# david-zwicker/video-analysis

Measured on AMD Instinct MI355X. Metric: frames/sec (bg-sub+blur+thresh+CCL) 1080p uint8, higher is better.
Workload: dtype u8; 1 GPU; cfg3_1080p_full_chain: 1920x1080 uint8, batch 256/GPU, running-mean bg-sub (f64 state) + sigma=5 Gaussian (q8.8) + threshold 20 + 5x5 dilate/erode + 4-connected labelling + object counts; inputs resident in HBM; engine=bg=1 gauss=mfma-i8(ksize=31) thresh=20 morph=2 ccl=4, video=one clip per rank, overlap=off, world_size=1, backend=single process

## Files before the change

video-analysis_amd/csrc/va_morph.hip:

```cpp
#include <math.h>

#include "va_common.h"

namespace va {

int make_row_spans(int shape, int ksize, RowSpans *out)
{
    VA_REQUIRE(ksize >= 1, "morphology: ksize must be >= 1 (got %d)", ksize);
    if (ksize > 63) {
        set_error("morphology: ksize %d > 63 is not supported", ksize);
        return VA_ERR_RANGE;
    }
    VA_REQUIRE(shape >= VA_SHAPE_RECT && shape <= VA_SHAPE_ELLIPSE, "morphology: bad shape %d",
               shape);
    out->ksize = ksize;
    out->anchor = ksize / 2;
    const int r = ksize / 2, c = ksize / 2;
    const double inv_r2 = r ? 1.0 / ((double)r * r) : 0.0;
    for (int i = 0; i < ksize; i++) {
        int j1 = 0, j2 = 0;
        if (shape == VA_SHAPE_RECT || (shape == VA_SHAPE_CROSS && i == r)) {
            j2 = ksize;
        } else if (shape == VA_SHAPE_CROSS) {
            j1 = c;
            j2 = j1 + 1;
        } else {
            int dy = i - r;
            if (abs(dy) <= r) {
                int dx = (int)lrint(c * sqrt((r * r - dy * dy) * inv_r2));
                j1 = c - dx > 0 ? c - dx : 0;
                j2 = c + dx + 1 < ksize ? c + dx + 1 : ksize;
            }
        }
        out->lo[i] = (int8_t)j1;
        out->hi[i] = (int8_t)j2;
    }
    return VA_OK;
}

namespace {

constexpr int kBlock = 256;

__global__ void __launch_bounds__(kBlock)
pack_bits_kernel(const uint8_t *__restrict__ src, uint32_t *__restrict__ bits, int w, int w32,
                 size_t total_words, int thresh, int vec_ok)
{
    size_t t = (size_t)blockIdx.x * kBlock + threadIdx.x;
    if (t >= total_words)
        return;
    int wi = (int)(t % w32);
    size_t rowi = t / w32;
    const uint8_t *p = src + rowi * (size_t)w + (size_t)wi * 32;
    int nvalid = w - wi * 32;
    nvalid = nvalid > 32 ? 32 : nvalid;
    uint32_t m = 0;
    if (vec_ok && nvalid == 32) {
        uint4 a = reinterpret_cast<const uint4 *>(p)[0];
        uint4 b = reinterpret_cast<const uint4 *>(p)[1];
        uint8_t px[32];
        memcpy(px, &a, 16);
        memcpy(px + 16, &b, 16);
#pragma unroll
        for (int k = 0; k < 32; k++)
            m |= (uint32_t)((int)px[k] > thresh) << k;
    } else {
        for (int k = 0; k < nvalid; k++)
            m |= (uint32_t)((int)p[k] > thresh) << k;
    }
    bits[t] = m;
}

__global__ void __launch_bounds__(kBlock)
unpack_bits_wide_kernel(const uint32_t *__restrict__ bits, uint8_t *__restrict__ dst, size_t total_halves,
                        int maxval)
{
    const size_t t = (size_t)blockIdx.x * kBlock + threadIdx.x;
    if (t >= total_halves)
        return;
    const uint32_t m = (bits[t >> 1] >> (16 * (t & 1))) & 0xFFFFu;
    typedef unsigned int v4u __attribute__((ext_vector_type(4)));
    v4u v;
#pragma unroll
    for (int q = 0; q < 4; q++)
        v[q] = ((((m >> (4 * q)) & 0xFu) * 0x00204081u) & 0x01010101u) * (uint32_t)maxval;
    __builtin_nontemporal_store(v, reinterpret_cast<v4u *>(dst + 16 * t));
}

__global__ void __launch_bounds__(kBlock)
unpack_bits_kernel(const uint32_t *__restrict__ bits, uint8_t *__restrict__ dst, int w, int w32,
                   size_t total_words, int maxval, int vec_ok)
{
    size_t t = (size_t)blockIdx.x * kBlock + threadIdx.x;
    if (t >= total_words)
        return;
    int wi = (int)(t % w32);
    size_t rowi = t / w32;
    uint8_t *p = dst + rowi * (size_t)w + (size_t)wi * 32;
    int nvalid = w - wi * 32;
    nvalid = nvalid > 32 ? 32 : nvalid;
    uint32_t m = bits[t];
    if (vec_ok && nvalid == 32) {
        uint8_t px[32];
#pragma unroll
        for (int k = 0; k < 32; k++)
            px[k] = (m >> k) & 1u ? (uint8_t)maxval : (uint8_t)0;
        uint4 a, b;
        memcpy(&a, px, 16);
        memcpy(&b, px + 16, 16);
        reinterpret_cast<uint4 *>(p)[0] = a;
        reinterpret_cast<uint4 *>(p)[1] = b;
    } else {
        for (int k = 0; k < nvalid; k++)
            p[k] = (m >> k) & 1u ? (uint8_t)maxval : (uint8_t)0;
    }
}

template <bool DILATE>
__global__ void __launch_bounds__(kBlock)
morph_bits_kernel(const uint32_t *__restrict__ src, uint32_t *__restrict__ dst, int h, int w,
                  int w32, size_t total_words, RowSpans se)
{
    size_t t = (size_t)blockIdx.x * kBlock + threadIdx.x;
    if (t >= total_words)
        return;
    const int wi = (int)(t % w32);
    const size_t rowi = t / w32;
    const int y = (int)(rowi % h);
    const uint32_t *frame = src + (rowi - y) * (size_t)w32;
    const uint32_t border = DILATE ? 0u : 0xFFFFFFFFu;
    const int tail = w & 31;
    const uint32_t last_valid = tail ? (0xFFFFFFFFu >> (32 - tail)) : 0xFFFFFFFFu;
    uint32_t acc = border;
    for (int i = 0; i < se.ksize; i++) {
        const int yy = y + i - se.anchor;
        if (yy < 0 || yy >= h)
            continue;
        const int lo = se.lo[i] - se.anchor, hi = se.hi[i] - 1 - se.anchor;
        if (lo > hi)
            continue;
        const uint32_t *row = frame + (size_t)yy * w32;
        uint32_t c = row[wi];
        uint32_t l = wi > 0 ? row[wi - 1] : border;
        uint32_t r = wi + 1 < w32 ? row[wi + 1] : border;
        if (!DILATE) {
            if (wi == w32 - 1)
                c |= ~last_valid;
            if (wi + 1 == w32 - 1)
                r |= ~last_valid;
        }
        uint32_t racc = border;
        for (int dx = lo; dx <= hi; dx++) {
            uint32_t s;
            if (dx == 0)
                s = c;
            else if (dx > 0)
                s = (c >> dx) | (r << (32 - dx));
            else
                s = (c << -dx) | (l >> (32 + dx));
            racc = DILATE ? (racc | s) : (racc & s);
        }
        acc = DILATE ? (acc | racc) : (acc & racc);
    }
    if (wi == w32 - 1)
        acc &= last_valid;
    dst[t] = acc;
}

struct MorphSeq {
    int count;
    int reach_total;
    int op[VA_MAX_MORPH_OPS];
    RowSpans se[VA_MAX_MORPH_OPS];
};
constexpr int kBandRows = 32;

__device__ __forceinline__ uint32_t morph_word_lds(const uint32_t *buf, int rbase, int y, int wi,
                                                  int h, int w32, uint32_t last_valid,
                                                  const RowSpans &se, bool dilate)
{
    const uint32_t border = dilate ? 0u : 0xFFFFFFFFu;
    uint32_t acc = border;
    for (int i = 0; i < se.ksize; i++) {
        const int yy = y + i - se.anchor;
        if (yy < 0 || yy >= h)
            continue;
        const int lo = se.lo[i] - se.anchor, hi = se.hi[i] - 1 - se.anchor;
        if (lo > hi)
            continue;
        const uint32_t *row = buf + (size_t)(yy - rbase) * w32;
        uint32_t c = row[wi];
        uint32_t l = wi > 0 ? row[wi - 1] : border;
        uint32_t r = wi + 1 < w32 ? row[wi + 1] : border;
        if (!dilate) {
            if (wi == w32 - 1)
                c |= ~last_valid;
            if (wi + 1 == w32 - 1)
                r |= ~last_valid;
        }
        uint32_t racc = border;
        for (int dx = lo; dx <= hi; dx++) {
            uint32_t sft;
            if (dx == 0)
                sft = c;
            else if (dx > 0)
                sft = (c >> dx) | (r << (32 - dx));
            else
                sft = (c << -dx) | (l >> (32 + dx));
            racc = dilate ? (racc | sft) : (racc & sft);
        }
        acc = dilate ? (acc | racc) : (acc & racc);
    }
    if (wi == w32 - 1)
        acc &= last_valid;
    return acc;
}

__device__ __forceinline__ uint32_t shift_words(uint32_t l, uint32_t c, uint32_t r, int dx)
{
    if (dx == 0)
        return c;
    return dx > 0 ? __builtin_amdgcn_alignbit(r, c, dx) : __builtin_amdgcn_alignbit(c, l, 32 + dx);
}

__global__ void __launch_bounds__(kBlock)
morph_fused_kernel(const uint32_t *__restrict__ src, uint32_t *__restrict__ dst, int h, int w, int w32, int nbands, MorphSeq seq)
{
    extern __shared__ uint32_t s_rows[];
    const int band = blockIdx.x % nbands, f = blockIdx.x / nbands;
    const int tx = threadIdx.x & 63, ty = threadIdx.x >> 6;
    const int y0 = band * kBandRows;
    const int nrows = kBandRows + 2 * seq.reach_total;
    const int rbase = y0 - seq.reach_total;
    uint32_t *bufA = s_rows, *bufB = s_rows + (size_t)nrows * w32, *bufH = bufB + (size_t)nrows * w32;
    const uint32_t *fsrc = src + (size_t)f * h * w32;
    const int tail = w & 31;
    const uint32_t last_valid = tail ? (0xFFFFFFFFu >> (32 - tail)) : 0xFFFFFFFFu;

    for (int wi = tx; wi < w32; wi += 64) {
        for (int r0 = ty; r0 < nrows; r0 += 32) {
            uint32_t tmp[8];
#pragma unroll
            for (int j = 0; j < 8; j++) {
                const int r = r0 + 4 * j, y = rbase + r;
                tmp[j] = (r < nrows && y >= 0 && y < h) ? fsrc[(size_t)y * w32 + wi] : 0u;
            }
#pragma unroll
            for (int j = 0; j < 8; j++) {
                const int r = r0 + 4 * j;
                if (r < nrows)
                    bufA[r * w32 + wi] = tmp[j];
            }
        }
    }
    __syncthreads();

    int reach = 0;
    for (int k = 0; k < seq.count; k++) {
        const RowSpans &se = seq.se[k];
        const int a = se.anchor, b = se.ksize - 1 - se.anchor;
        reach += a > b ? a : b;
        const int lo = max(0, rbase + reach), hi = min(h, rbase + nrows - reach);
        const bool dil = seq.op[k] == VA_MORPH_DILATE;
        const uint32_t border = dil ? 0u : 0xFFFFFFFFu;
        bool rect = true;
        for (int i = 1; i < se.ksize; i++)
            rect = rect && se.lo[i] == se.lo[0] && se.hi[i] == se.hi[0];
        rect = rect && se.lo[0] < se.hi[0];
        if (rect) {
            const int dlo = se.lo[0] - a, dhi = se.hi[0] - 1 - a;
            const int ylo = max(0, lo - a), yhi = min(h, hi + b);
            for (int y = ylo + ty; y < yhi; y += 4) {
                const uint32_t *row = bufA + (y - rbase) * w32;
                for (int wi = tx; wi < w32; wi += 64) {
                    uint32_t c = row[wi];
                    uint32_t l = wi > 0 ? row[wi - 1] : border;
                    uint32_t r = wi + 1 < w32 ? row[wi + 1] : border;
                    if (!dil) {
                        if (wi == w32 - 1)
                            c |= ~last_valid;
                        if (wi + 1 == w32 - 1)
                            r |= ~last_valid;
                    }
                    uint32_t racc = border;
                    for (int dx = dlo; dx <= dhi; dx++) {
                        const uint32_t sft = shift_words(l, c, r, dx);
                        racc = dil ? (racc | sft) : (racc & sft);
                    }
                    bufH[(y - rbase) * w32 + wi] = racc;
                }
            }
            __syncthreads();
            for (int y = lo + ty; y < hi; y += 4) {
                const int i0 = max(0, a - y), i1 = min(se.ksize, h + a - y);
                for (int wi = tx; wi < w32; wi += 64) {
                    uint32_t acc = border;
                    for (int i = i0; i < i1; i++) {
                        const uint32_t v = bufH[(y + i - a - rbase) * w32 + wi];
                        acc = dil ? (acc | v) : (acc & v);
                    }
                    if (wi == w32 - 1)
                        acc &= last_valid;
                    bufB[(y - rbase) * w32 + wi] = acc;
                }
            }
        } else {
            for (int y = lo + ty; y < hi; y += 4)
                for (int wi = tx; wi < w32; wi += 64)
                    bufB[(y - rbase) * w32 + wi] =
                        morph_word_lds(bufA, rbase, y, wi, h, w32, last_valid, se, dil);
        }
        __syncthreads();
        uint32_t *t = bufA;
        bufA = bufB;
        bufB = t;
    }

    const int yend = min(h, y0 + kBandRows);
    uint32_t *fdst = dst + (size_t)f * h * w32;
    for (int y = y0 + ty; y < yend; y += 4) {
        const uint32_t *row = bufA + (y - rbase) * w32;
        for (int wi = tx; wi < w32; wi += 64)
            fdst[(size_t)y * w32 + wi] = row[wi];
    }
}

constexpr int kStreamBand = 32;

template <int K>
__device__ __forceinline__ uint32_t hdilate(uint32_t l, uint32_t c, uint32_t r)
{
    uint32_t acc = c;
#pragma unroll
    for (int d = 1; d <= K / 2; d++) {
        acc |= __builtin_amdgcn_alignbit(r, c, d);
        acc |= __builtin_amdgcn_alignbit(c, l, 32 - d);
    }
    return acc;
}

constexpr int kStreamGroup = 8;

__device__ __forceinline__ uint32_t lane_left(uint32_t v)
{
    return __builtin_amdgcn_update_dpp(0u, v, 0x138 , 0xf, 0xf, true);
}
__device__ __forceinline__ uint32_t lane_right(uint32_t v)
{
    return __builtin_amdgcn_update_dpp(0u, v, 0x130 , 0xf, 0xf, true);
}

template <int K0, int K1>
__global__ void __launch_bounds__(kBlock)
morph_stream_kernel(const uint32_t *__restrict__ src, uint32_t *__restrict__ dst, int n, int h, int w,
                     int w32, int nbands, int nchunks, uint32_t flip_in, uint32_t flip_mid,
                     uint32_t flip_out)
{
    constexpr int A0 = K0 / 2, A1 = K1 / 2;
    constexpr int LO = K1 ? 2 : 1;
    constexpr int COLS = K1 ? 60 : 62;
    const int lane = threadIdx.x & 63;
    size_t item = (size_t)blockIdx.x * (kBlock / 64) + (threadIdx.x >> 6);
    const int chunk = (int)(item % nchunks);
    item /= nchunks;
    const int band = (int)(item % nbands);
    const size_t f = item / nbands;
    if (f >= (size_t)n)
        return;
    const int wi = chunk * COLS + lane - LO;
    const bool col_in = wi >= 0 && wi < w32;
    const bool col_store = col_in && lane >= LO && lane < LO + COLS;
    const int tail = w & 31;
    const uint32_t valid = !col_in ? 0u : (wi == w32 - 1 && tail ? (0xFFFFFFFFu >> (32 - tail)) : 0xFFFFFFFFu);
    const uint32_t *fsrc = src + f * (size_t)h * w32 + min(max(wi, 0), w32 - 1);
    uint32_t *fdst = dst + f * (size_t)h * w32;

    const int y0 = band * kStreamBand;
    if (y0 >= h)
        return;
    const int y_first = y0 - A0 - A1;
    const int y_last = min(h, y0 + kStreamBand) - 1 + A0 + A1;

    auto load_group = [&](int y, uint32_t (&g)[kStreamGroup]) {
#pragma unroll
        for (int k = 0; k < kStreamGroup; k++)
            g[k] = fsrc[(size_t)min(max(y + k, 0), h - 1) * w32];
#pragma unroll
        for (int k = 0; k < kStreamGroup; k++)
            g[k] = (y + k >= 0 && y + k < h) ? ((g[k] ^ flip_in) & valid) : 0u;
    };

    uint32_t win0[K0], win1[K1 ? K1 : 1];
#pragma unroll
    for (int k = 0; k < K0; k++)
        win0[k] = 0u;
#pragma unroll
    for (int k = 0; k < (K1 ? K1 : 1); k++)
        win1[k] = 0u;

    uint32_t cur[kStreamGroup], nxt[kStreamGroup];
    load_group(y_first, nxt);
    for (int yg = y_first; yg <= y_last; yg += kStreamGroup) {
#pragma unroll
        for (int k = 0; k < kStreamGroup; k++)
            cur[k] = nxt[k];
        if (yg + kStreamGroup <= y_last)
            load_group(yg + kStreamGroup, nxt);
#pragma unroll
        for (int k = 0; k < kStreamGroup; k++) {
            const int y = yg + k;
            if (y > y_last)
                break;
            const uint32_t c = cur[k], l = lane_left(c), r = lane_right(c);
#pragma unroll
            for (int j = 0; j + 1 < K0; j++)
                win0[j] = win0[j + 1];
            win0[K0 - 1] = hdilate<K0>(l, c, r);
            uint32_t v0 = 0u;
#pragma unroll
            for (int j = 0; j < K0; j++)
                v0 |= win0[j];
            const int ya = y - A0;
            uint32_t out;
            int yo;
            if constexpr (K1 == 0) {
                out = (v0 ^ flip_out) & valid;
                yo = ya;
            } else {
                const uint32_t t = (ya >= 0 && ya < h) ? ((v0 ^ flip_mid) & valid) : 0u;
                const uint32_t tl = lane_left(t), tr = lane_right(t);
#pragma unroll
                for (int j = 0; j + 1 < K1; j++)
                    win1[j] = win1[j + 1];
                win1[K1 ? K1 - 1 : 0] = hdilate<(K1 ? K1 : 1)>(tl, t, tr);
                uint32_t v1 = 0u;
#pragma unroll
                for (int j = 0; j < K1; j++)
                    v1 |= win1[j];
                out = (v1 ^ flip_out) & valid;
                yo = ya - A1;
            }
            if (col_store && yo >= y0 && yo < y0 + kStreamBand && yo < h)
                fdst[(size_t)yo * w32 + wi] = out;
        }
    }
}

template <bool DILATE>
__global__ void __launch_bounds__(kBlock)
morph_u8_kernel(const uint8_t *__restrict__ src, uint8_t *__restrict__ dst, int h, int w,
                size_t total, RowSpans se)
{
    size_t e = (size_t)blockIdx.x * kBlock + threadIdx.x;
    if (e >= total)
        return;
    const int x = (int)(e % w);
    const size_t rowi = e / w;
    const int y = (int)(rowi % h);
    const uint8_t *frame = src + (rowi - y) * (size_t)w;
    int best = DILATE ? 0 : 255;
    for (int i = 0; i < se.ksize; i++) {
        const int yy = y + i - se.anchor;
        if (yy < 0 || yy >= h)
            continue;
        int x0 = x + se.lo[i] - se.anchor, x1 = x + se.hi[i] - 1 - se.anchor;
        x0 = x0 < 0 ? 0 : x0;
        x1 = x1 >= w ? w - 1 : x1;
        const uint8_t *row = frame + (size_t)yy * w;
        for (int xx = x0; xx <= x1; xx++) {
            int v = row[xx];
            best = DILATE ? (v > best ? v : best) : (v < best ? v : best);
        }
    }
    dst[e] = (uint8_t)best;
}

inline bool aligned(const void *p, size_t a) { return (reinterpret_cast<uintptr_t>(p) % a) == 0; }

}

int launch_pack_bits(const uint8_t *src, uint32_t *bits, int n, int h, int w, int thresh,
                     hipStream_t st)
{
    const int w32 = words_per_row(w);
    size_t total = (size_t)n * h * w32;
    if (total == 0)
        return VA_OK;
    int vec = (w % 32 == 0) && aligned(src, 16);
    pack_bits_kernel<<<cdiv((long long)total, kBlock), kBlock, 0, st>>>(src, bits, w, w32, total,
                                                                       thresh, vec);
    VA_LAUNCH_CHECK("pack_bits_kernel");
    return VA_OK;
}

int launch_unpack_bits(const uint32_t *bits, uint8_t *dst, int n, int h, int w, int maxval,
                       hipStream_t st)
{
    const int w32 = words_per_row(w);
    size_t total = (size_t)n * h * w32;
    if (total == 0)
        return VA_OK;
    int vec = (w % 32 == 0) && aligned(dst, 16);
    if (vec)
        unpack_bits_wide_kernel<<<cdiv((long long)(2 * total), kBlock), kBlock, 0, st>>>(bits, dst, 2 * total,
                                                                                         maxval);
    else
        unpack_bits_kernel<<<cdiv((long long)total, kBlock), kBlock, 0, st>>>(bits, dst, w, w32, total,
                                                                             maxval, vec);
    VA_LAUNCH_CHECK("unpack_bits_kernel");
    return VA_OK;
}

int launch_morph_bits(const uint32_t *src, uint32_t *dst, int n, int h, int w, int op,
                      const RowSpans &se, hipStream_t st)
{
    const int w32 = words_per_row(w);
    size_t total = (size_t)n * h * w32;
    if (total == 0)
        return VA_OK;
    int grid = cdiv((long long)total, kBlock);
    if (op == VA_MORPH_DILATE)
        morph_bits_kernel<true><<<grid, kBlock, 0, st>>>(src, dst, h, w, w32, total, se);
    else
        morph_bits_kernel<false><<<grid, kBlock, 0, st>>>(src, dst, h, w, w32, total, se);
    VA_LAUNCH_CHECK("morph_bits_kernel");
    return VA_OK;
}

bool morph_fused_supported(int w, const RowSpans *se, int count)
{
    if (count < 1 || count > VA_MAX_MORPH_OPS)
        return false;
    int reach = 0;
    for (int k = 0; k < count; k++) {
        int a = se[k].anchor, b = se[k].ksize - 1 - se[k].anchor;
        reach += a > b ? a : b;
    }
    size_t lds = 3 * (size_t)(kBandRows + 2 * reach) * words_per_row(w) * sizeof(uint32_t);
    return reach <= 16 && lds <= 64 * 1024;
}

static bool is_rect_odd(const RowSpans &se, int kmax)
{
    if (!(se.ksize & 1) || se.ksize > kmax || se.ksize < 3)
        return false;
    for (int i = 0; i < se.ksize; i++)
        if (se.lo[i] != 0 || se.hi[i] != se.ksize)
            return false;
    return true;
}

template <int K0, int K1>
static int launch_stream(const uint32_t *src, uint32_t *dst, int n, int h, int w, const int *ops,
                         hipStream_t st)
{
    const int w32 = words_per_row(w);
    const int cols = K1 ? 60 : 62;
    const int nchunks = cdiv(w32, cols), nbands = cdiv(h, kStreamBand);
    const size_t items = (size_t)n * nbands * nchunks;
    const uint32_t e0 = ops[0] == VA_MORPH_ERODE ? 0xFFFFFFFFu : 0u;
    const uint32_t e1 = K1 ? (ops[1] == VA_MORPH_ERODE ? 0xFFFFFFFFu : 0u) : 0u;
    const uint32_t flip_in = e0, flip_mid = e0 ^ e1, flip_out = K1 ? e1 : e0;
    const int waves_per_block = kBlock / 64;
    const size_t blocks = (items + waves_per_block - 1) / waves_per_block;
    morph_stream_kernel<K0, K1><<<(unsigned)blocks, kBlock, 0, st>>>(
        src, dst, n, h, w, w32, nbands, nchunks, flip_in, flip_mid, flip_out);
    VA_LAUNCH_CHECK("morph_stream_kernel");
    return VA_OK;
}

int launch_morph_fused(const uint32_t *src, uint32_t *dst, int n, int h, int w, const int *ops,
                       const RowSpans *se, int count, hipStream_t st)
{
    VA_REQUIRE(morph_fused_supported(w, se, count), "fused morphology: unsupported sequence");
    if (n == 0 || h == 0 || w == 0)
        return VA_OK;
    if (count <= 2 && is_rect_odd(se[0], 7) && (count == 1 || is_rect_odd(se[1], 7))) {
        const int k0 = se[0].ksize, k1 = count == 2 ? se[1].ksize : 0;
#define VA_STREAM_CASE(A, B) \
    if (k0 == A && k1 == B)  \
        return launch_stream<A, B>(src, dst, n, h, w, ops, st);
        VA_STREAM_CASE(3, 0) VA_STREAM_CASE(5, 0) VA_STREAM_CASE(7, 0)
        VA_STREAM_CASE(3, 3) VA_STREAM_CASE(3, 5) VA_STREAM_CASE(3, 7)
        VA_STREAM_CASE(5, 3) VA_STREAM_CASE(5, 5) VA_STREAM_CASE(5, 7)
        VA_STREAM_CASE(7, 3) VA_STREAM_CASE(7, 5) VA_STREAM_CASE(7, 7)
#undef VA_STREAM_CASE
    }
    MorphSeq seq;
    memset(&seq, 0, sizeof(seq));
    seq.count = count;
    for (int k = 0; k < count; k++) {
        seq.op[k] = ops[k];
        seq.se[k] = se[k];
        int a = se[k].anchor, b = se[k].ksize - 1 - se[k].anchor;
        seq.reach_total += a > b ? a : b;
    }
    const int w32 = words_per_row(w);
    const int nbands = cdiv(h, kBandRows);
    const size_t lds = 3 * (size_t)(kBandRows + 2 * seq.reach_total) * w32 * sizeof(uint32_t);
    morph_fused_kernel<<<nbands * n, kBlock, lds, st>>>(src, dst, h, w, w32, nbands,
                                                       seq);
    VA_LAUNCH_CHECK("morph_fused_kernel");
    return VA_OK;
}

template <bool DILATE, bool VERT>
__global__ void __launch_bounds__(kBlock)
morph_u8_line_kernel(const uint8_t *__restrict__ src, uint8_t *__restrict__ dst, int h, int w, size_t total,
                     int ksize, int anchor)
{
    size_t e = (size_t)blockIdx.x * kBlock + threadIdx.x;
    if (e >= total)
        return;
    const int x = (int)(e % w);
    const size_t rowi = e / w;
    const int y = (int)(rowi % h);
    const uint8_t *frame = src + (rowi - y) * (size_t)w;
    int best = DILATE ? 0 : 255;
    const int c = VERT ? y : x, len = VERT ? h : w;
    int a = c - anchor, b = c - anchor + ksize - 1;
    a = a < 0 ? 0 : a;
    b = b >= len ? len - 1 : b;
    for (int t = a; t <= b; t++) {
        const int v = VERT ? frame[(size_t)t * w + x] : frame[(size_t)y * w + t];
        best = DILATE ? (v > best ? v : best) : (v < best ? v : best);
    }
    dst[e] = (uint8_t)best;
}

namespace {

typedef unsigned short us2 __attribute__((ext_vector_type(2)));
template <bool DILATE>
struct Extreme4 {
    us2 even, odd;
    __device__ __forceinline__ Extreme4()
    {
        const unsigned short v = DILATE ? 0 : 255;
        even = us2{v, v};
        odd = us2{v, v};
    }
    __device__ __forceinline__ void take(uint32_t d)
    {
        const us2 e = __builtin_bit_cast(us2, d & 0x00FF00FFu), o = __builtin_bit_cast(us2, (d >> 8) & 0x00FF00FFu);
        even = DILATE ? __builtin_elementwise_max(even, e) : __builtin_elementwise_min(even, e);
        odd = DILATE ? __builtin_elementwise_max(odd, o) : __builtin_elementwise_min(odd, o);
    }
    __device__ __forceinline__ uint32_t word() const
    {
        return __builtin_bit_cast(uint32_t, even) | (__builtin_bit_cast(uint32_t, odd) << 8);
    }
};

template <bool DILATE>
__global__ void __launch_bounds__(kBlock)
morph_u8_rows_x4_kernel(const uint8_t *__restrict__ src, uint8_t *__restrict__ dst, int h, int w, RowSpans se)
{
    const int q = blockIdx.x * kBlock + threadIdx.x, wq = w >> 2;
    if (q >= wq)
        return;
    const int y = blockIdx.y;
    const size_t f = blockIdx.z;
    const uint32_t *frame = reinterpret_cast<const uint32_t *>(src + f * (size_t)h * w);
    const uint32_t neutral = DILATE ? 0u : 0xFFFFFFFFu;
    Extreme4<DILATE> best;
    for (int i = 0; i < se.ksize; i++) {
        const int yy = y + i - se.anchor;
        const int lo = se.lo[i], hi = se.hi[i];
        if (yy < 0 || yy >= h || hi <= lo)
            continue;
        const uint32_t *row = frame + (size_t)yy * wq;
        int off = lo - se.anchor;
        int d = q + (off >> 2);
        uint32_t cur = (d >= 0 && d < wq) ? row[d] : neutral;
        uint32_t nxt = (d + 1 >= 0 && d + 1 < wq) ? row[d + 1] : neutral;
        for (int s = lo; s < hi; s++, off++) {
            const int sh = off & 3;
            if (sh == 0 && s != lo) {
                d++;
                cur = nxt;
                nxt = (d + 1 >= 0 && d + 1 < wq) ? row[d + 1] : neutral;
            }
            best.take(__builtin_amdgcn_alignbyte(nxt, cur, sh));
        }
    }
    reinterpret_cast<uint32_t *>(dst + (f * h + y) * (size_t)w)[q] = best.word();
}

template <bool DILATE>
__global__ void __launch_bounds__(kBlock)
morph_u8_vert_x4_kernel(const uint8_t *__restrict__ src, uint8_t *__restrict__ dst, int h, int w, int ksize, int anchor)
{
    const int q = blockIdx.x * kBlock + threadIdx.x, wq = w >> 2;
    if (q >= wq)
        return;
    const int y = blockIdx.y;
    const size_t f = blockIdx.z;
    const uint32_t *frame = reinterpret_cast<const uint32_t *>(src + f * (size_t)h * w);
    int a = y - anchor, b = y - anchor + ksize - 1;
    a = a < 0 ? 0 : a;
    b = b >= h ? h - 1 : b;
    Extreme4<DILATE> best;
    for (int t = a; t <= b; t++)
        best.take(frame[(size_t)t * wq + q]);
    reinterpret_cast<uint32_t *>(dst + (f * h + y) * (size_t)w)[q] = best.word();
}

}

int launch_morph_u8(const uint8_t *src, uint8_t *dst, int n, int h, int w, int op,
                    const RowSpans &se, hipStream_t st, uint8_t *scratch)
{
    if (w % 4 == 0 && h <= 65535 && n <= 65535 && n > 0 && src != dst && reinterpret_cast<uintptr_t>(src) % 4 == 0 &&
        reinterpret_cast<uintptr_t>(dst) % 4 == 0 && (!scratch || reinterpret_cast<uintptr_t>(scratch) % 4 == 0)) {
        const dim3 grid((unsigned)cdiv(w / 4, kBlock), (unsigned)h, (unsigned)n);
        bool full = scratch != nullptr && se.ksize >= 3;
        for (int i = 0; i < se.ksize && full; i++)
            full = se.lo[i] == 0 && se.hi[i] == se.ksize;
        if (full) {
            RowSpans line = {};
            line.ksize = 1;
            line.anchor = 0;
            line.lo[0] = (int8_t)(-se.anchor);
            line.hi[0] = (int8_t)(se.ksize - se.anchor);
            if (op == VA_MORPH_DILATE) {
                morph_u8_rows_x4_kernel<true><<<grid, kBlock, 0, st>>>(src, scratch, h, w, line);
                morph_u8_vert_x4_kernel<true><<<grid, kBlock, 0, st>>>(scratch, dst, h, w, se.ksize, se.anchor);
            } else {
                morph_u8_rows_x4_kernel<false><<<grid, kBlock, 0, st>>>(src, scratch, h, w, line);
                morph_u8_vert_x4_kernel<false><<<grid, kBlock, 0, st>>>(scratch, dst, h, w, se.ksize, se.anchor);
            }
        } else if (op == VA_MORPH_DILATE) {
            morph_u8_rows_x4_kernel<true><<<grid, kBlock, 0, st>>>(src, dst, h, w, se);
        } else {
            morph_u8_rows_x4_kernel<false><<<grid, kBlock, 0, st>>>(src, dst, h, w, se);
        }
        VA_LAUNCH_CHECK("morph_u8_x4 kernels");
        return VA_OK;
    }
    bool rect = scratch != nullptr && se.ksize >= 3;
    for (int i = 0; i < se.ksize && rect; i++)
        rect = se.lo[i] == 0 && se.hi[i] == se.ksize;
    if (rect) {
        size_t total = (size_t)n * h * w;
        if (total == 0)
            return VA_OK;
        const int grid = cdiv((long long)total, kBlock);
        if (op == VA_MORPH_DILATE) {
            morph_u8_line_kernel<true, false><<<grid, kBlock, 0, st>>>(src, scratch, h, w, total, se.ksize, se.anchor);
            morph_u8_line_kernel<true, true><<<grid, kBlock, 0, st>>>(scratch, dst, h, w, total, se.ksize, se.anchor);
        } else {
            morph_u8_line_kernel<false, false><<<grid, kBlock, 0, st>>>(src, scratch, h, w, total, se.ksize, se.anchor);
            morph_u8_line_kernel<false, true><<<grid, kBlock, 0, st>>>(scratch, dst, h, w, total, se.ksize, se.anchor);
        }
        VA_LAUNCH_CHECK("morph_u8_line_kernel");
        return VA_OK;
    }

    size_t total = (size_t)n * h * w;
    if (total == 0)
        return VA_OK;
    int grid = cdiv((long long)total, kBlock);
    if (op == VA_MORPH_DILATE)
        morph_u8_kernel<true><<<grid, kBlock, 0, st>>>(src, dst, h, w, total, se);
    else
        morph_u8_kernel<false><<<grid, kBlock, 0, st>>>(src, dst, h, w, total, se);
    VA_LAUNCH_CHECK("morph_u8_kernel");
    return VA_OK;
}

}
```

Measured before the change: 317,300 frames/s.

## Restructure streaming morphology with buffer loads, ring windows and interior-band fast path

Reworks the fused streaming dilate/erode kernel. It sizes the row group and band height so the band plus halo divides evenly into groups, and replaces shift-register windows with modular ring indexing where the group size is a multiple of the kernel size. Row loads and stores now go through raw buffer descriptors whose size is zeroed for out-of-range rows, which replaces clamped addressing and per-row branches. It also adds a fully unrolled path for interior bands without boundary checks and a launch-bounds occupancy hint. The costs are larger code, more register pressure from full unrolling and the doubled group buffer, and reliance on buffer out-of-bounds semantics for correctness.

```diff
diff --git a/video-analysis_amd/csrc/va_morph.hip b/video-analysis_amd/csrc/va_morph.hip
--- a/video-analysis_amd/csrc/va_morph.hip
+++ b/video-analysis_amd/csrc/va_morph.hip
@@ -1,4 +1,6 @@
 #include <math.h>
+
+#include <type_traits>
 
 #include "va_common.h"
 
@@ -325,8 +327,6 @@
     }
 }
 
-constexpr int kStreamBand = 32;
-
 template <int K>
 __device__ __forceinline__ uint32_t hdilate(uint32_t l, uint32_t c, uint32_t r)
 {
@@ -339,7 +339,20 @@
     return acc;
 }
 
-constexpr int kStreamGroup = 8;
+template <int K0, int K1>
+constexpr int stream_group()
+{
+    return (K1 != 0 && K1 != K0) ? 8 : K0 == 3 ? 9 : K0 == 5 ? 10 : 7;
+}
+
+template <int K0, int K1>
+constexpr int stream_band()
+{
+    int b = 32;
+    while ((b + 2 * (K0 / 2 + K1 / 2)) % stream_group<K0, K1>())
+        b++;
+    return b;
+}
 
 __device__ __forceinline__ uint32_t lane_left(uint32_t v)
 {
@@ -350,44 +363,66 @@
     return __builtin_amdgcn_update_dpp(0u, v, 0x130 , 0xf, 0xf, true);
 }
 
+__device__ __forceinline__ __amdgpu_buffer_rsrc_t row_rsrc(uintptr_t row, uint32_t bytes)
+{
+    return __builtin_amdgcn_make_buffer_rsrc(reinterpret_cast<void *>(row), 0, (int)bytes, 0x00027000);
+}
+
 template <int K0, int K1>
-__global__ void __launch_bounds__(kBlock)
+__global__ void __launch_bounds__(kBlock, 8)
 morph_stream_kernel(const uint32_t *__restrict__ src, uint32_t *__restrict__ dst, int n, int h, int w,
                      int w32, int nbands, int nchunks, uint32_t flip_in, uint32_t flip_mid,
                      uint32_t flip_out)
 {
-    constexpr int A0 = K0 / 2, A1 = K1 / 2;
+    constexpr int A0 = K0 / 2, A1 = K1 / 2, R = A0 + A1;
+    constexpr int G = stream_group<K0, K1>();
+    constexpr int band_rows = stream_band<K0, K1>(), kSteps = (band_rows + 2 * R) / G;
+    constexpr bool kFixed0 = G % K0 == 0, kFixed1 = K1 && G % (K1 ? K1 : 1) == 0;
     constexpr int LO = K1 ? 2 : 1;
     constexpr int COLS = K1 ? 60 : 62;
+    constexpr uint32_t kOob = 0xFFFFFFFFu;
     const int lane = threadIdx.x & 63;
-    size_t item = (size_t)blockIdx.x * (kBlock / 64) + (threadIdx.x >> 6);
-    const int chunk = (int)(item % nchunks);
-    item /= nchunks;
-    const int band = (int)(item % nbands);
-    const size_t f = item / nbands;
-    if (f >= (size_t)n)
+    uint32_t item = blockIdx.x * (uint32_t)(kBlock / 64) +
+                    (uint32_t)__builtin_amdgcn_readfirstlane((int)(threadIdx.x >> 6));
+    const int chunk = (int)(item % (uint32_t)nchunks);
+    item /= (uint32_t)nchunks;
+    const int band = (int)(item % (uint32_t)nbands);
+    const int f = (int)(item / (uint32_t)nbands);
+    if (f >= n)
         return;
+    const int y0 = band * band_rows;
+    const int yend = min(h, y0 + band_rows);
+    const int y_first = y0 - R;
+    const int y_last = yend - 1 + R;
+    const uint32_t row_bytes = (uint32_t)w32 * 4u;
+
     const int wi = chunk * COLS + lane - LO;
     const bool col_in = wi >= 0 && wi < w32;
     const bool col_store = col_in && lane >= LO && lane < LO + COLS;
     const int tail = w & 31;
     const uint32_t valid = !col_in ? 0u : (wi == w32 - 1 && tail ? (0xFFFFFFFFu >> (32 - tail)) : 0xFFFFFFFFu);
-    const uint32_t *fsrc = src + f * (size_t)h * w32 + min(max(wi, 0), w32 - 1);
-    uint32_t *fdst = dst + f * (size_t)h * w32;
-
-    const int y0 = band * kStreamBand;
-    if (y0 >= h)
-        return;
-    const int y_first = y0 - A0 - A1;
-    const int y_last = min(h, y0 + kStreamBand) - 1 + A0 + A1;
-
-    auto load_group = [&](int y, uint32_t (&g)[kStreamGroup]) {
-#pragma unroll
-        for (int k = 0; k < kStreamGroup; k++)
-            g[k] = fsrc[(size_t)min(max(y + k, 0), h - 1) * w32];
-#pragma unroll
-        for (int k = 0; k < kStreamGroup; k++)
-            g[k] = (y + k >= 0 && y + k < h) ? ((g[k] ^ flip_in) & valid) : 0u;
+    const uint32_t ld_off = col_in ? (uint32_t)wi * 4u : kOob;
+    const uint32_t st_off = col_store ? (uint32_t)wi * 4u : kOob;
+
+    const long long frow = (long long)f * h;
+    uintptr_t ld_row = reinterpret_cast<uintptr_t>(src) + (uintptr_t)((frow + y_first) * (long long)row_bytes);
+    uintptr_t st_row = reinterpret_cast<uintptr_t>(dst) + (uintptr_t)((frow + y_first - R) * (long long)row_bytes);
+
+    const bool band_interior = y_first >= A0 && y_last < h && yend - y0 == band_rows;
+
+    auto next_row = [&](uintptr_t &row) {
+        row += row_bytes;
+        asm("" : "+s"(row));
+    };
+
+    auto load_group = [&](auto interior_c, int yg, uint32_t (&g)[G]) {
+        constexpr bool INTERIOR = decltype(interior_c)::value;
+#pragma unroll
+        for (int k = 0; k < G; k++, next_row(ld_row)) {
+            uint32_t bytes = (INTERIOR || (yg + k >= 0 && yg + k <= min(h - 1, y_last))) ? row_bytes : 0u;
+            asm("" : "+s"(bytes));
+            g[k] = __builtin_amdgcn_raw_buffer_load_b32(row_rsrc(ld_row, bytes), ld_off, 0, 0);
+        }
     };
 
     uint32_t win0[K0], win1[K1 ? K1 : 1];
@@ -398,52 +433,73 @@
     for (int k = 0; k < (K1 ? K1 : 1); k++)
         win1[k] = 0u;
 
-    uint32_t cur[kStreamGroup], nxt[kStreamGroup];
-    load_group(y_first, nxt);
-    for (int yg = y_first; yg <= y_last; yg += kStreamGroup) {
-#pragma unroll
-        for (int k = 0; k < kStreamGroup; k++)
-            cur[k] = nxt[k];
-        if (yg + kStreamGroup <= y_last)
-            load_group(yg + kStreamGroup, nxt);
-#pragma unroll
-        for (int k = 0; k < kStreamGroup; k++) {
+    auto rows = [&](auto interior_c, int yg, const uint32_t (&cur)[G]) {
+        constexpr bool INTERIOR = decltype(interior_c)::value;
+#pragma unroll
+        for (int k = 0; k < G; k++) {
             const int y = yg + k;
-            if (y > y_last)
-                break;
-            const uint32_t c = cur[k], l = lane_left(c), r = lane_right(c);
-#pragma unroll
-            for (int j = 0; j + 1 < K0; j++)
-                win0[j] = win0[j + 1];
-            win0[K0 - 1] = hdilate<K0>(l, c, r);
+            const uint32_t in_ok = (INTERIOR || (y >= 0 && y < h)) ? 0xFFFFFFFFu : 0u;
+            const uint32_t c = (cur[k] ^ flip_in) & (INTERIOR ? valid : (valid & in_ok));
+            const uint32_t l = lane_left(c), r = lane_right(c);
+            if constexpr (kFixed0) {
+                win0[k % K0] = hdilate<K0>(l, c, r);
+            } else {
+#pragma unroll
+                for (int j = 0; j + 1 < K0; j++)
+                    win0[j] = win0[j + 1];
+                win0[K0 - 1] = hdilate<K0>(l, c, r);
+            }
             uint32_t v0 = 0u;
 #pragma unroll
             for (int j = 0; j < K0; j++)
                 v0 |= win0[j];
-            const int ya = y - A0;
             uint32_t out;
-            int yo;
             if constexpr (K1 == 0) {
                 out = (v0 ^ flip_out) & valid;
-                yo = ya;
             } else {
-                const uint32_t t = (ya >= 0 && ya < h) ? ((v0 ^ flip_mid) & valid) : 0u;
+                const int ya = y - A0;
+                const uint32_t mid_ok = (INTERIOR || (ya >= 0 && ya < h)) ? 0xFFFFFFFFu : 0u;
+                const uint32_t t = (v0 ^ flip_mid) & (INTERIOR ? valid : (valid & mid_ok));
                 const uint32_t tl = lane_left(t), tr = lane_right(t);
-#pragma unroll
-                for (int j = 0; j + 1 < K1; j++)
-                    win1[j] = win1[j + 1];
-                win1[K1 ? K1 - 1 : 0] = hdilate<(K1 ? K1 : 1)>(tl, t, tr);
+                if constexpr (kFixed1) {
+                    win1[k % (K1 ? K1 : 1)] = hdilate<(K1 ? K1 : 1)>(tl, t, tr);
+                } else {
+#pragma unroll
+                    for (int j = 0; j + 1 < K1; j++)
+                        win1[j] = win1[j + 1];
+                    win1[K1 ? K1 - 1 : 0] = hdilate<(K1 ? K1 : 1)>(tl, t, tr);
+                }
                 uint32_t v1 = 0u;
 #pragma unroll
                 for (int j = 0; j < K1; j++)
                     v1 |= win1[j];
                 out = (v1 ^ flip_out) & valid;
-                yo = ya - A1;
             }
-            if (col_store && yo >= y0 && yo < y0 + kStreamBand && yo < h)
-                fdst[(size_t)yo * w32 + wi] = out;
-        }
-    }
+            const bool st_ok = y - R >= y0 && (INTERIOR || y <= y_last);
+            uint32_t bytes = st_ok ? row_bytes : 0u;
+            asm("" : "+s"(bytes));
+            __builtin_amdgcn_raw_buffer_store_b32(out, row_rsrc(st_row, bytes), st_off, 0, 0);
+            next_row(st_row);
+        }
+    };
+
+    auto march = [&](auto interior_c) {
+        uint32_t g[2][G];
+        load_group(interior_c, y_first, g[0]);
+#pragma unroll
+        for (int s = 0; s < kSteps; s++) {
+            const int yg = y_first + s * G;
+            if (yg > y_last)
+                break;
+            if (s + 1 < kSteps)
+                load_group(interior_c, yg + G, g[(s + 1) & 1]);
+            rows(interior_c, yg, g[s & 1]);
+        }
+    };
+    if (band_interior)
+        march(std::true_type{});
+    else
+        march(std::false_type{});
 }
 
 template <bool DILATE>
@@ -556,13 +612,15 @@
 {
     const int w32 = words_per_row(w);
     const int cols = K1 ? 60 : 62;
-    const int nchunks = cdiv(w32, cols), nbands = cdiv(h, kStreamBand);
+    const int nchunks = cdiv(w32, cols);
+    const int nbands = cdiv(h, stream_band<K0, K1>());
     const size_t items = (size_t)n * nbands * nchunks;
     const uint32_t e0 = ops[0] == VA_MORPH_ERODE ? 0xFFFFFFFFu : 0u;
     const uint32_t e1 = K1 ? (ops[1] == VA_MORPH_ERODE ? 0xFFFFFFFFu : 0u) : 0u;
     const uint32_t flip_in = e0, flip_mid = e0 ^ e1, flip_out = K1 ? e1 : e0;
     const int waves_per_block = kBlock / 64;
     const size_t blocks = (items + waves_per_block - 1) / waves_per_block;
+    VA_REQUIRE(blocks <= 0x3FFFFFFFu, "streaming morphology: too many bands (%zu waves)", items);
     morph_stream_kernel<K0, K1><<<(unsigned)blocks, kBlock, 0, st>>>(
         src, dst, n, h, w, w32, nbands, nchunks, flip_in, flip_mid, flip_out);
     VA_LAUNCH_CHECK("morph_stream_kernel");
```

Result: no change. 319,000 frames/s (median of 6 runs) (+0.5%).
